# Baverne/VAE-CYCLEGAN-Implementation

Hardware: AMD Instinct MI355X
Metric: train images/sec (256x256 VAE-CycleGAN step) (higher is better)
Workload: dtype f32; 1 GPU; cyclevaegan unpaired, 3x256x256 synthetic summer<->winter, per-GPU batch 8, latent 64 (BASELINE.json configs[3]/[4]); per_gpu_batch=8, global_batch=8, image_size=256, latent_dim=64, parallelism=dp1, init=random (reference init statistics)

## Files before the change

vae-cyclegan-implementation_amd/csrc/conv_igemm.hip:

```cpp
#include "vcg_common.h"
#ifdef VCG_STAMP
#include <stdlib.h>
#endif

struct ConvP {
  const float* a;
  const float* b;
  const float* bias;
  float* out;
  int N, H, W, Cin, Cout, KH, KW, stride, pad, reflect, ups, act;
  int Hl, Wl, Ho, Wo, M, K;
  int cin4, cout4, cout_log;
  FastDiv fd_howo, fd_wo, fd_cin4, fd_cout4, fd_kw, fd_cin;
  int Hc, Wc, Mc, NB;
  FastDiv fd_hcwc, fd_wc;
  int ktiles_total, sk_len, sk_units, sk_ntn, sk_bm_shift, sk_bn_shift;
  int sk_ntr_pb;
  FastDiv fd_sklen;
  int ksplit, kt_per;
  float* slab;
  int adjoint;
  int src_pitch;
  uint32_t a_bytes, b_bytes;
  int dbl_mirror;
// ... 590 lines not shown
  f32x16 acc[MI][NI], tot[MI][NI];
#pragma unroll
  for (int i = 0; i < MI; ++i)
#pragma unroll
    for (int j = 0; j < NI; ++j)
#pragma unroll
      for (int e = 0; e < 16; ++e) acc[i][j][e] = tot[i][j][e] = 0.f;

  float4 va[AR], ve[AR], vb[BR];
  int nkt = (Kc + BK - 1) / BK;
  int kt0 = 0;
  if (p.ksplit > 1) {
    kt0 = kslice * p.kt_per;
    int kt1 = kt0 + p.kt_per;
    nkt = kt1 < nkt ? kt1 : nkt;
  }

  const __amdgpu_buffer_rsrc_t ra = make_srd(p.a, p.a_bytes), rb = make_srd(p.b, p.b_bytes);
  const int NONE = -(1 << 20);
  int eh[AR], ew[AR];
  bool edge[AR], any_edge = false;
#pragma unroll
  for (int r = 0; r < AR; ++r) {
    const int h = ph[r], w = pw[r];
    eh[r] = (h >= 1 && h <= p.pad) ? -h : (h >= p.Hl - 1 - p.pad && h <= p.Hl - 2) ? 2 * (p.Hl - 1) - h : NONE;
    ew[r] = (w >= 1 && w <= p.pad) ? -w : (w >= p.Wl - 1 - p.pad && w <= p.Wl - 2) ? 2 * (p.Wl - 1) - w : NONE;
    edge[r] = pv[r] && p.reflect && (eh[r] != NONE || ew[r] != NONE);
    any_edge = any_edge || edge[r];
    ve[r] = f4zero();
  }
  uint32_t rowoff[AR], xoff[AR][3], wbase[BR];
  int tap_cur = -1;

  auto load_tiles = [&](int kt) {
    const uint32_t g = (uint32_t)(kt * 8 + a_u);
    const bool kv = (int)(g * 4) < Kc;
    const uint32_t tapc = fd_div(g, p.fd_cout4);
    const int co = (int)(g - tapc * (uint32_t)p.cout4) * 4;
    if ((int)tapc != tap_cur) {
      tap_cur = (int)tapc;
      const int u = (int)tapc / nKW, v_ = (int)tapc % nKW;
      const int kh = kh0 + u * s, kw = kw0 + v_ * s;
      auto src = [&](int r, int qh, int qw) -> uint32_t {
        const int numh = qh - kh + p.pad, numw = qw - kw + p.pad;
        const int oh = numh >> sshift, ow = numw >> sshift;
        const bool ok = pv[r] && qh != NONE && qw != NONE && numh >= 0 && oh < p.Ho && numw >= 0 && ow < p.Wo;
        return ok ? (uint32_t)(((pnHo[r] + oh) * p.Wo + ow) * p.Cout) * 4u : VCG_OOB;
      };
#pragma unroll
      for (int r = 0; r < AR; ++r) {
        rowoff[r] = src(r, ph[r], pw[r]);
        if (any_edge) {
          xoff[r][0] = edge[r] ? src(r, eh[r], pw[r]) : VCG_OOB;
          xoff[r][1] = edge[r] ? src(r, ph[r], ew[r]) : VCG_OOB;
          xoff[r][2] = edge[r] ? src(r, eh[r], ew[r]) : VCG_OOB;
        }
      }
      const int tapfull = kh * p.KW + kw;
#pragma unroll
      for (int r = 0; r < BR; ++r) {
        const int J = n0 + a_row + 32 * r;
        wbase[r] = J < p.NB ? (uint32_t)((tapfull * p.NB + J) * p.Cout) * 4u : VCG_OOB;
      }
    }
    const uint32_t cb4 = (uint32_t)co * 4u;
#pragma unroll
    for (int r = 0; r < AR; ++r) va[r] = bload4(ra, (kv && rowoff[r] != VCG_OOB) ? rowoff[r] + cb4 : VCG_OOB);
    if (p.dbl_mirror) {
      const int u = tap_cur / nKW, v_ = tap_cur % nKW;
#pragma unroll
      for (int r = 0; r < AR; ++r)
        ve[r] = (pv[r] && kv) ? adjoint_extras(p, p.a, pnHo[r], ph[r], pw[r], kh0 + u * s, kw0 + v_ * s, co, sshift) : f4zero();
    } else if (any_edge) {
#pragma unroll
      for (int r = 0; r < AR; ++r) {
        float4 e = f4zero();
        if (edge[r] && kv) {
#pragma unroll
          for (int k = 0; k < 3; ++k)
            if (xoff[r][k] != VCG_OOB) f4add(e, bload4(ra, xoff[r][k] + cb4));
        }
        ve[r] = e;
      }
    }
#pragma unroll
    for (int r = 0; r < BR; ++r) vb[r] = bload4(rb, (kv && wbase[r] != VCG_OOB) ? wbase[r] + cb4 : VCG_OOB);
  };
  auto store_tiles = [&](int buf) {
#pragma unroll
    for (int r = 0; r < AR; ++r) {
      float* d = &As[buf][(a_row + 32 * r) * AS_STRIDE + a_u * 4];
      d[0] = va[r].x + ve[r].x; d[1] = va[r].y + ve[r].y; d[2] = va[r].z + ve[r].z; d[3] = va[r].w + ve[r].w;
    }
#pragma unroll
    for (int r = 0; r < BR; ++r) {
      float* d = &Bt[buf][(a_row + 32 * r) * AS_STRIDE + a_u * 4];
      d[0] = vb[r].x; d[1] = vb[r].y; d[2] = vb[r].z; d[3] = vb[r].w;
    }
  };

  if (kt0 < nkt) {
    load_tiles(kt0);
    store_tiles(0);
  }
  __syncthreads();
  VCG_STAMP_AT(1);
  for (int kt = kt0; kt < nkt; ++kt) {
    const int cur = (kt - kt0) & 1;
    const float* const Ac = As[cur];
    const float* const Bc = Bt[cur];
    if (kt + 1 < nkt) load_tiles(kt + 1);
    mma_ktile<MI, NI>(
        acc, [&](int kk, int i) { return Ac[(wm * (BM / WM) + i * 32 + l31) * AS_STRIDE + kk]; },
        [&](int kk, int j) { return Bc[(wn * (BN / WN) + j * 32 + l31) * AS_STRIDE + kk]; }, lh);
    if (((kt - kt0 + 1) & (FLUSH_TILES - 1)) == 0 && kt + 1 < nkt) flush_acc<MI, NI>(acc, tot);
    if (kt + 1 < nkt) store_tiles(cur ^ 1);
    __syncthreads();
  }
  VCG_STAMP_AT(2);
#pragma unroll
  for (int i = 0; i < MI; ++i)
#pragma unroll
    for (int j = 0; j < NI; ++j) acc[i][j] += tot[i][j];

  float* const dst = p.ksplit > 1 ? p.slab + (size_t)kslice * p.N * p.H * p.W * p.Cin : p.out;
#pragma unroll
  for (int j = 0; j < NI; ++j) {
    const int J = n0 + wn * (BN / WN) + j * 32 + l31;
    if (J >= p.NB) continue;
    int q = 0, c = J;
    if (p.ups == 2) { q = (int)fd_div((uint32_t)J, p.fd_cin); c = J - q * p.Cin; }
    const int qi = q >> 1, qj = q & 1;
#pragma unroll
    for (int i = 0; i < MI; ++i) {
#pragma unroll
      for (int e = 0; e < 16; ++e) {
        const int row = (e & 3) + 8 * (e >> 2) + 4 * lh;
        const uint32_t m = (uint32_t)(m0 + wm * (BM / WM) + i * 32 + row);
        if (m < (uint32_t)p.Mc) {
          uint32_t n = fd_div(m, p.fd_hcwc);
          uint32_t rem = m - n * (uint32_t)(p.Hc * p.Wc);
          uint32_t hq = fd_div(rem, p.fd_wc);
          uint32_t wq = rem - hq * (uint32_t)p.Wc;
          int h = (int)hq * s + ca, w = (int)wq * s + cb;
          size_t off = ((size_t)((int)n * p.H + h * p.ups + qi) * p.W + (w * p.ups + qj)) * p.Cin + c;
          dst[off] = acc[i][j][e];
        }
      }
    }
  }
  VCG_STAMP_AT(3);
}

template <int BN, int WN, bool BPL = (BN >= 64)>
__global__ __launch_bounds__(256, 2) void k_conv_dgrad_split(ConvP p) {
  VCG_STAMP_AT(0);
  constexpr int BM = 128, WM = 4 / WN;
  constexpr int MI = BM / (32 * WM), NI = BN / (32 * WN), AR = BM / 32, BR = BN / 32;
  __shared__ __attribute__((aligned(16))) unsigned char As[VCG_NP][BM * 64];
  __shared__ __attribute__((aligned(16))) unsigned char Bs[VCG_NP][BN * 64];
  const int tid = threadIdx.x, lane = tid & 63, wid = tid >> 6;
  const int wm = wid / WN, wn = wid % WN, l31 = lane & 31, lh = lane >> 5;
  const SplitScales sc = split_scales(p);
  const int m0 = blockIdx.x * BM, n0 = blockIdx.y * BN;
  const int a_row = tid >> 3, a_u = tid & 7;
  const int s = p.stride, sshift = s - 1;
  const int cls = (int)blockIdx.z % (s * s), kslice = (int)blockIdx.z / (s * s);
  const int ca = cls / s, cb = cls % s;
  const int kh0 = (ca + p.pad) % s, kw0 = (cb + p.pad) % s;
  const int nKH = (p.KH - kh0 + s - 1) / s, nKW = (p.KW - kw0 + s - 1) / s;
  const int Kc = nKH * nKW * p.Cout;

  int pnHo[AR], ph[AR], pw[AR];
  bool pv[AR];
#pragma unroll
  for (int r = 0; r < AR; ++r) {
    uint32_t m = (uint32_t)(m0 + a_row + 32 * r);
    pv[r] = m < (uint32_t)p.Mc;
    uint32_t n = fd_div(m, p.fd_hcwc);
    uint32_t rem = m - n * (uint32_t)(p.Hc * p.Wc);
    uint32_t hq = fd_div(rem, p.fd_wc);
    uint32_t wq = rem - hq * (uint32_t)p.Wc;
    pnHo[r] = (int)n * p.Ho;
    ph[r] = (int)hq * s + ca;
    pw[r] = (int)wq * s + cb;
  }

  f32x16 acc[MI][NI], lo[MI][NI];
#pragma unroll
  for (int i = 0; i < MI; ++i)
#pragma unroll
    for (int j = 0; j < NI; ++j)
#pragma unroll
      for (int e = 0; e < 16; ++e) acc[i][j][e] = lo[i][j][e] = 0.f;

  float4 va[AR], ve[AR], vb[BPL ? 1 : BR];
  constexpr int BP = BPL ? VCG_NP * BN / 64 : 1;
  const int b_q = tid & 3, b_r = tid >> 2;
  const int CB = p.Cout / 32;
  const uint32_t bsoff0 = (uint32_t)(b_r * 64 + ((b_q ^ ((b_r >> 2) & 3)) << 4));
  u32x4 vbp[BP];
  int nkt = (Kc + BK - 1) / BK;
  int kt0 = 0;
  if (p.ksplit > 1) {
    kt0 = kslice * p.kt_per;
    int kt1 = kt0 + p.kt_per;
    nkt = kt1 < nkt ? kt1 : nkt;
  }

  const __amdgpu_buffer_rsrc_t ra = make_srd(p.a, p.a_bytes), rb = make_srd(p.b, p.b_bytes);
  const int NONE = -(1 << 20);
  int eh[AR], ew[AR];
  bool edge[AR], any_edge = false;
#pragma unroll
  for (int r = 0; r < AR; ++r) {
    const int h = ph[r], w = pw[r];
    eh[r] = (h >= 1 && h <= p.pad) ? -h : (h >= p.Hl - 1 - p.pad && h <= p.Hl - 2) ? 2 * (p.Hl - 1) - h : NONE;
    ew[r] = (w >= 1 && w <= p.pad) ? -w : (w >= p.Wl - 1 - p.pad && w <= p.Wl - 2) ? 2 * (p.Wl - 1) - w : NONE;
    edge[r] = pv[r] && p.reflect && (eh[r] != NONE || ew[r] != NONE);
    any_edge = any_edge || edge[r];
    ve[r] = f4zero();
  }
  uint32_t rowoff[AR], xoff[AR][3], wbase[BR];
  int tap_cur = -1;

  auto load_tiles = [&](int kt) {
    const uint32_t g = (uint32_t)(kt * 8 + a_u);
    const bool kv = (int)(g * 4) < Kc;
    const uint32_t tapc = fd_div(g, p.fd_cout4);
    const int co = (int)(g - tapc * (uint32_t)p.cout4) * 4;
    if ((int)tapc != tap_cur) {
      tap_cur = (int)tapc;
      const int u = (int)tapc / nKW, v_ = (int)tapc % nKW;
      const int kh = kh0 + u * s, kw = kw0 + v_ * s;
      auto src = [&](int r, int qh, int qw) -> uint32_t {
        const int numh = qh - kh + p.pad, numw = qw - kw + p.pad;
        const int oh = numh >> sshift, ow = numw >> sshift;
        const bool ok = pv[r] && qh != NONE && qw != NONE && numh >= 0 && oh < p.Ho && numw >= 0 && ow < p.Wo;
        return ok ? (uint32_t)(((pnHo[r] + oh) * p.Wo + ow) * p.Cout) * 4u : VCG_OOB;
      };
#pragma unroll
      for (int r = 0; r < AR; ++r) {
        rowoff[r] = src(r, ph[r], pw[r]);
        if (any_edge) {
          xoff[r][0] = edge[r] ? src(r, eh[r], pw[r]) : VCG_OOB;
          xoff[r][1] = edge[r] ? src(r, ph[r], ew[r]) : VCG_OOB;
          xoff[r][2] = edge[r] ? src(r, eh[r], ew[r]) : VCG_OOB;
        }
      }
      const int tapfull = kh * p.KW + kw;
      if constexpr (!BPL) {
#pragma unroll
        for (int r = 0; r < BR; ++r) {
          const int J = n0 + a_row + 32 * r;
          wbase[r] = J < p.NB ? (uint32_t)((tapfull * p.NB + J) * p.Cout) * 4u : VCG_OOB;
        }
      }
    }
    const uint32_t cb4 = (uint32_t)co * 4u;
#pragma unroll
    for (int r = 0; r < AR; ++r) va[r] = bload4(ra, (kv && rowoff[r] != VCG_OOB) ? rowoff[r] + cb4 : VCG_OOB);
    if (p.dbl_mirror) {
      const int u = tap_cur / nKW, v_ = tap_cur % nKW;
#pragma unroll
      for (int r = 0; r < AR; ++r)
        ve[r] = (pv[r] && kv) ? adjoint_extras(p, p.a, pnHo[r], ph[r], pw[r], kh0 + u * s, kw0 + v_ * s, co, sshift) : f4zero();
    } else if (any_edge) {
#pragma unroll
      for (int r = 0; r < AR; ++r) {
        float4 e = f4zero();
        if (edge[r] && kv) {
#pragma unroll
          for (int k = 0; k < 3; ++k)
            if (xoff[r][k] != VCG_OOB) f4add(e, bload4(ra, xoff[r][k] + cb4));
        }
        ve[r] = e;
      }
    }
    if constexpr (BPL) {
      const int tk = (kt * 32) / p.Cout, cob = (kt * 32 - tk * p.Cout) >> 5;
      const int tf = (kh0 + (tk / nKW) * s) * p.KW + (kw0 + (tk % nKW) * s);
      const bool kvt = kt * 32 < Kc;
#pragma unroll
      for (int j = 0; j < BP; ++j) {
        const int J = n0 + b_r + 64 * (j / VCG_NP);
        const uint32_t off = (kvt && J < p.NB) ? (uint32_t)((((size_t)tf * p.NB + J) * CB + cob) * VCG_PBYTES + (j % VCG_NP) * 64 + b_q * 16) : VCG_OOB;
        vbp[j] = __builtin_amdgcn_raw_buffer_load_b128(rb, (int)off, 0, 0);
      }
    } else {
#pragma unroll
      for (int r = 0; r < BR; ++r) vb[r] = bload4(rb, (kv && wbase[r] != VCG_OOB) ? wbase[r] + cb4 : VCG_OOB);
    }
  };
  uint32_t soff[AR > BR ? AR : BR];
#pragma unroll
  for (int i = 0; i < (AR > BR ? AR : BR); ++i) {
    const int r = a_row + 32 * i;
    soff[i] = (uint32_t)(r * 64 + (((a_u >> 1) ^ ((r >> 2) & 3)) << 4) + ((a_u & 1) << 3));
  }
  auto store_tiles = [&]() {
#pragma unroll
    for (int r = 0; r < AR; ++r) {
      const float4 v = make_float4(va[r].x + ve[r].x, va[r].y + ve[r].y, va[r].z + ve[r].z, va[r].w + ve[r].w);
      uint2 h, l;
      split4h(v, sc.inv_a, h, l);
      *reinterpret_cast<uint2*>(&As[0][soff[r]]) = h;
      *reinterpret_cast<uint2*>(&As[1][soff[r]]) = l;
    }
    if constexpr (BPL) {
#pragma unroll
      for (int j = 0; j < BP; ++j) *reinterpret_cast<u32x4*>(&Bs[j % VCG_NP][bsoff0 + 4096 * (j / VCG_NP)]) = vbp[j];
    } else {
#pragma unroll
      for (int r = 0; r < BR; ++r) {
        uint2 h, l;
        split4h(vb[r], sc.inv_b, h, l);
        *reinterpret_cast<uint2*>(&Bs[0][soff[r]]) = h;
        *reinterpret_cast<uint2*>(&Bs[1][soff[r]]) = l;
      }
    }
  };
  uint32_t fa[MI], fb[NI];
  int sa[MI], sb[NI];
#pragma unroll
  for (int i = 0; i < MI; ++i) { const int r = wm * (BM / WM) + i * 32 + l31; fa[i] = (uint32_t)(r * 64); sa[i] = (r >> 2) & 3; }
#pragma unroll
  for (int j = 0; j < NI; ++j) { const int r = wn * (BN / WN) + j * 32 + l31; fb[j] = (uint32_t)(r * 64); sb[j] = (r >> 2) & 3; }

  if (kt0 < nkt) {
    load_tiles(kt0);
    store_tiles();
  }
  __syncthreads();
  VCG_STAMP_AT(1);
  for (int kt = kt0; kt < nkt; ++kt) {
    if (kt + 1 < nkt) load_tiles(kt + 1);
    split_mma_ktile<MI, NI>(acc, lo, As, Bs, fa, fb, sa, sb, lh);
    __syncthreads();
    if (kt + 1 < nkt) {
      store_tiles();
      __syncthreads();
    }
  }
  VCG_STAMP_AT(2);
#pragma unroll
  for (int i = 0; i < MI; ++i)
#pragma unroll
    for (int j = 0; j < NI; ++j) acc[i][j] += lo[i][j];

  float* const dst = p.ksplit > 1 ? p.slab + (size_t)kslice * p.N * p.H * p.W * p.Cin : p.out;
#pragma unroll
  for (int j = 0; j < NI; ++j) {
    const int J = n0 + wn * (BN / WN) + j * 32 + l31;
    if (J >= p.NB) continue;
    int q = 0, c = J;
    if (p.ups == 2) { q = (int)fd_div((uint32_t)J, p.fd_cin); c = J - q * p.Cin; }
    const int qi = q >> 1, qj = q & 1;
#pragma unroll
    for (int i = 0; i < MI; ++i) {
#pragma unroll
      for (int e = 0; e < 16; ++e) {
        const int row = (e & 3) + 8 * (e >> 2) + 4 * lh;
        const uint32_t m = (uint32_t)(m0 + wm * (BM / WM) + i * 32 + row);
        if (m < (uint32_t)p.Mc) {
          uint32_t n = fd_div(m, p.fd_hcwc);
          uint32_t rem = m - n * (uint32_t)(p.Hc * p.Wc);
          uint32_t hq = fd_div(rem, p.fd_wc);
          uint32_t wq = rem - hq * (uint32_t)p.Wc;
          int h = (int)hq * s + ca, w = (int)wq * s + cb;
          size_t off = ((size_t)((int)n * p.H + h * p.ups + qi) * p.W + (w * p.ups + qj)) * p.Cin + c;
          dst[off] = acc[i][j][e] * sc.out;
        }
      }
    }
  }
  VCG_STAMP_AT(3);
}

__device__ __forceinline__ int sk_logical_wg() {
  const uint32_t nwg = gridDim.x, gid = blockIdx.x;
  const uint32_t q = nwg >> 3, r = nwg & 7, xcd = gid & 7;
  return (int)((xcd < r ? xcd * (q + 1) : r * (q + 1) + (xcd - r) * q) + (gid >> 3));
}

template <int BM, int BN, int NT = 256>
__global__ __launch_bounds__(NT) void k_conv_wgrad(ConvP p) {
  VCG_STAMP_AT(0);
  constexpr int WR = NT / 128;
  constexpr int MI = BM / (32 * WR), NI = BN / 64;
  constexpr int RQ = BM / 4, PS = NT / RQ, AP = BK / PS, BE = (BK * BN / 4) / NT;
  __shared__ __attribute__((aligned(16))) float Xs[2][BK * BM];
  __shared__ __attribute__((aligned(16))) float Ds[2][BK * BN];
  const int tid = threadIdx.x, lane = tid & 63, wid = tid >> 6;
  const int wm = wid >> 1, wn = wid & 1, l31 = lane & 31, lh = lane >> 5;
  const int rq = tid % RQ, ps = tid / RQ;
  const uint32_t bstep = (uint32_t)(BK * p.Cout * 4);
  const bool row_aligned = !p.adjoint && (p.Wo % BK) == 0;

  const int wg = sk_logical_wg();
  int unit = wg * p.sk_len;
  int unit_end = unit + p.sk_len;
  if (unit_end > p.sk_units) unit_end = p.sk_units;
  while (unit < unit_end) {
  const int tile = unit / p.ktiles_total;
  const int kt_begin = unit - tile * p.ktiles_total;
  int kt_end = kt_begin + (unit_end - unit);
  if (kt_end > p.ktiles_total) kt_end = p.ktiles_total;
  const int tr = tile / p.sk_ntn;
  const int zb = tr / p.sk_ntr_pb;
  const int r0 = (tr - zb * p.sk_ntr_pb) * BM, n0 = (tile - tr * p.sk_ntn) * BN;
  const __amdgpu_buffer_rsrc_t ra = make_srd(p.a + (size_t)zb * p.a_bstride, p.a_bytes),
                               rb = make_srd(p.b + (size_t)zb * p.b_bstride, p.b_bytes);

  const int R = r0 + rq * 4;
  const bool rv = R < p.K;
  int kh, kw, ii, jj, c;
  decode_tap(p, (uint32_t)(R >> 2), kh, kw, ii, jj, c);

  f32x16 acc[MI][NI];
#pragma unroll
  for (int i = 0; i < MI; ++i)
#pragma unroll
    for (int j = 0; j < NI; ++j)
#pragma unroll
      for (int e = 0; e < 16; ++e) acc[i][j][e] = 0.f;

  float4 va[AP], vb[BE];

  uint32_t sm[AP];
  int sn[AP], soh[AP], sow[AP];
#pragma unroll
  for (int a = 0; a < AP; ++a) {
    uint32_t m = (uint32_t)(kt_begin * BK + ps + PS * a);
    uint32_t n = fd_div(m, p.fd_howo);
    uint32_t rem = m - n * (uint32_t)(p.Ho * p.Wo);
    uint32_t oh = fd_div(rem, p.fd_wo);
    sm[a] = m; sn[a] = (int)n; soh[a] = (int)oh; sow[a] = (int)(rem - oh * (uint32_t)p.Wo);
  }
  uint32_t boff[BE];
#pragma unroll
  for (int e = 0; e < BE; ++e) {
    int idx = tid + NT * e;
    int pp = idx / (BN / 4), j4 = idx % (BN / 4);
    const int co = n0 + j4 * 4;
    boff[e] = co < p.Cout ? (uint32_t)(((kt_begin * BK + pp) * p.Cout + co) * 4) : VCG_OOB;
  }

  auto load_tiles = [&](int ) {
    if (row_aligned) {
      const int n = sn[0], oh = soh[0];
      int ih = oh * p.stride - p.pad + kh;
      bool okr = rv && sm[0] < (uint32_t)p.M;
      if (p.reflect) ih = reflect_idx(ih, p.Hl);
      else okr = okr && ih >= 0 && ih < p.Hl;
      const uint32_t rowbase = (uint32_t)(((n * p.H + ih * p.ups + ii) * p.W + jj) * p.Cin + c) * 4u;
      const uint32_t colstep = (uint32_t)(p.ups * p.Cin) * 4u;
#pragma unroll
      for (int a = 0; a < AP; ++a) {
        int iw = sow[a] * p.stride - p.pad + kw;
        bool ok = okr;
        if (p.reflect) iw = reflect_idx(iw, p.Wl);
        else ok = ok && iw >= 0 && iw < p.Wl;
        va[a] = bload4(ra, ok ? rowbase + (uint32_t)iw * colstep : VCG_OOB);
        sm[a] += BK;
        sow[a] += BK;
        if (sow[a] >= p.Wo) { sow[a] -= p.Wo; ++soh[a]; if (soh[a] >= p.Ho) { soh[a] = 0; ++sn[a]; } }
      }
    } else {
#pragma unroll
      for (int a = 0; a < AP; ++a) {
        const int n = sn[a], oh = soh[a], ow = sow[a];
        if (p.adjoint) {
          float4 v = f4zero();
          if (rv && sm[a] < (uint32_t)p.M) {
            float4 ex;
            adjoint_gather(p, p.a, n * p.Ho, oh, ow, kh, kw, 0, 0, v, ex);
            f4add(v, ex);
          }
          va[a] = v;
        } else {
          int ih = oh * p.stride - p.pad + kh, iw = ow * p.stride - p.pad + kw;
          bool ok = rv && sm[a] < (uint32_t)p.M;
          if (p.reflect) {
            ih = reflect_idx(ih, p.Hl);
            iw = reflect_idx(iw, p.Wl);
          } else {
            ok = ok && (ih >= 0) && (ih < p.Hl) && (iw >= 0) && (iw < p.Wl);
          }
          const uint32_t off = ok ? (uint32_t)(((n * p.H + ih * p.ups + ii) * p.W + (iw * p.ups + jj)) * p.Cin + c) * 4u : VCG_OOB;
          va[a] = bload4(ra, off);
        }
        sm[a] += BK;
        sow[a] += BK;
        while (sow[a] >= p.Wo) { sow[a] -= p.Wo; ++soh[a]; }
        while (soh[a] >= p.Ho) { soh[a] -= p.Ho; ++sn[a]; }
      }
    }
#pragma unroll
    for (int e = 0; e < BE; ++e) {
      vb[e] = bload4(rb, boff[e]);
      if (boff[e] != VCG_OOB) boff[e] += bstep;
    }
  };
  auto store_tiles = [&](int buf) {
#pragma unroll
    for (int a = 0; a < AP; ++a)
      *reinterpret_cast<float4*>(&Xs[buf][(ps + PS * a) * BM + rq * 4]) = va[a];
#pragma unroll
    for (int e = 0; e < BE; ++e) {
      int idx = tid + NT * e;
      int pp = idx / (BN / 4), j4 = idx % (BN / 4);
      *reinterpret_cast<float4*>(&Ds[buf][pp * BN + j4 * 4]) = vb[e];
    }
  };

  if (kt_begin < kt_end) {
    load_tiles(kt_begin);
    store_tiles(0);
  }
  __syncthreads();
  VCG_STAMP_AT(1);
  for (int kt = kt_begin; kt < kt_end; ++kt) {
    const int cur = (kt - kt_begin) & 1;
    const float* const Xc = Xs[cur];
    const float* const Dc = Ds[cur];
    if (kt + 1 < kt_end) load_tiles(kt + 1);
    mma_ktile<MI, NI>(
        acc, [&](int kk, int i) { return Xc[kk * BM + wm * (BM / WR) + i * 32 + l31]; },
        [&](int kk, int j) { return Dc[kk * BN + wn * (BN / 2) + j * 32 + l31]; }, lh);
// ... 847 lines not shown
  int bm, bn, nsplit, kt_per;
  fwd_plan(g, bm, bn, nsplit, kt_per);
  return bm == 128 && bn >= 64 && nsplit == 1 && wft_wanted(g) && (g.Ho * g.Wo) % 128 == 0;
}

static int conv_fwd_impl(const float* x, const float* wf, const float* bias, float* y, const int32_t* cd, void* ws,
                         size_t ws_bytes, void* stream, double* in_part, const VcgInStatsOut* stats, float* saved = nullptr,
                         const VcgPre* pre = nullptr) {
  const uint64_t x_handle = vcg_take_hint_x();
  (void)vcg_take_hint_dy();
  ConvGeom g;
  if (vcg_conv_geom(cd, &g, "vcg_conv_fwd")) return -1;
  VCG_CHECK_ARG(x && wf && y, "vcg_conv_fwd: null pointer");
  if (pre && pre->mean)
    VCG_CHECK_ARG(!vcg_thin_fold_ok(g) && !vcg_thin_fwd_ok(g) && vcg_wino_fwd_ok(g),
                  "vcg_conv_fwd_in_pre: this geometry has no normalising gather (ask vcg_conv_pre_ok first)");
  if (vcg_thin_fold_ok(g)) return vcg_thin_fold_fwd(g, x, wf + wf_floats(g), vcg_pack_amax(g, wf), bias, y, ws, ws_bytes, (hipStream_t)stream, x_handle);
  if (vcg_thin_fwd_ok(g)) return vcg_thin_fwd(g, x, wf, bias, y, (hipStream_t)stream);
  if (vcg_thinin_fwd_ok(g)) {
    if (vcg_thinin_fwd(g, x, wf, vcg_pack_amax(g, wf), bias, y, in_part, (hipStream_t)stream, x_handle)) return -2;
    if (in_part)
      return vcg_in_finalize(in_part, stats->mean, stats->rstd, g.N, stats->HW, g.Cout, vcg_thinin_nchunk(g), stats->eps, (hipStream_t)stream);
    return 0;
  }
  if (vcg_wino_fwd_ok(g))
    return vcg_wino_fwd(g, x, wf + wf_floats(g), vcg_pack_amax(g, wf), bias, y, ws, ws_bytes, (hipStream_t)stream, in_part, stats, saved, x_handle,
                        pre);
  if (fwd_slab_ok(g))
    return vcg_slab_fwd(g, x, wf + wft_offset(g), wft_floats(g) * 4, vcg_pack_amax(g, wf), bias, y, in_part, stats, (hipStream_t)stream, x_handle);
  ConvP p; fill_params(g, p);
  if (in_part) {
    p.in_part = in_part;
    p.in_nchunk = g.Ho * g.Wo / 128;
  }
  p.a = x; p.b = wf; p.bias = bias; p.out = y;
  {
    const unsigned long long ab = (unsigned long long)g.N * g.H * g.W * g.Cin * 4, bb = (unsigned long long)g.K * g.Cout * 4;
    VCG_CHECK_ARG(ab < (1ull << 31) && bb < (1ull << 31), "vcg_conv_fwd: tensor extents must stay below 2 GiB");
    p.a_bytes = (uint32_t)ab; p.b_bytes = (uint32_t)bb;
  }
  int bm, bn, nsplit, kt_per;
  fwd_plan(g, bm, bn, nsplit, kt_per);
  if (nsplit > 1) {
    VCG_CHECK_ARG(ws && ws_bytes >= vcg_conv_fwd_workspace(cd), "vcg_conv_fwd: workspace too small (%zu)", ws_bytes);
    p.ksplit = nsplit; p.kt_per = kt_per; p.slab = (float*)ws;
  }
  dim3 grid((g.M + bm - 1) / bm, (g.Cout + bn - 1) / bn, nsplit);
  hipStream_t st = (hipStream_t)stream;
  const double gemm_flops = 2.0 * g.M * (double)g.K * g.Cout;
  if (bm == 128 && bn >= 64 && wft_wanted(g)) {
    p.b = wf + wft_offset(g);
    p.b_bytes = (uint32_t)(wft_floats(g) * 4);
    if (vcg_operand_amax(x, (size_t)g.N * g.H * g.W * g.Cin, x_handle, 0, st, &p.amax_a)) return -2;
    p.amax_b = vcg_amax_stored(vcg_pack_amax(g, wf));
    VcgProfScope prof(bn == 128 ? "k_conv_fwd_split<128>" : "k_conv_fwd_split<64>", gemm_flops, st);
    if (bn == 128) hipLaunchKernelGGL((k_conv_fwd_split<128>), grid, dim3(256), 0, st, p);
    else hipLaunchKernelGGL((k_conv_fwd_split<64>), grid, dim3(256), 0, st, p);
  } else {
    VcgProfScope prof("k_conv_fwd<fp32 MFMA>", gemm_flops, st);
    if (bm == 128 && bn == 128 && g.K <= 2048) hipLaunchKernelGGL((k_conv_fwd<128, 128, 2, false>), grid, dim3(256), 0, st, p);
    else DISPATCH_FWD(bm, bn, grid, st, p);
  }
  if (nsplit > 1)
    hipLaunchKernelGGL(k_splitk_finish, dim3(ew_grid((size_t)g.M * g.Cout / 4)), dim3(256), 0, st, (const float*)ws, bias,
                       y, (size_t)g.M, g.Cout, nsplit, g.cout_log, g.act);
  VCG_LAUNCH_CHECK("vcg_conv_fwd");
  if (in_part) return vcg_in_finalize(in_part, stats->mean, stats->rstd, g.N, stats->HW, g.Cout, p.in_nchunk, stats->eps, st);
  return 0;
}

extern "C" int vcg_conv_fwd(const float* x, const float* wf, const float* bias, float* y,
                            const int32_t* cd, void* ws, size_t ws_bytes, void* stream) {
  return conv_fwd_impl(x, wf, bias, y, cd, ws, ws_bytes, stream, nullptr, nullptr);
}

static size_t fwd_in_conv_ws(const int32_t* cd) { return (vcg_conv_fwd_workspace(cd) + 255) / 256 * 256; }

extern "C" size_t vcg_conv_fwd_in_workspace(const int32_t* cd) {
  ConvGeom g;
  if (vcg_conv_geom(cd, &g, "vcg_conv_fwd_in_workspace")) return 0;
  size_t part;
  const bool thinin = !vcg_thin_fold_ok(g) && !vcg_thin_fwd_ok(g) && vcg_thinin_fwd_ok(g);
  if (thinin) part = (size_t)g.N * vcg_thinin_nchunk(g) * g.Cout * 2 * sizeof(double);
  else if (vcg_wino_fwd_ok(g)) part = vcg_wino_fwd_stats_doubles(g) * sizeof(double);
  else if (fwd_slab_ok(g) && vcg_slab_fwd_stats_ok(g)) part = (size_t)g.N * vcg_slab_fwd_nchunk(g) * g.Cout * 2 * sizeof(double);
  else if (fwd_tile_stats_ok(g)) part = (size_t)g.N * (g.Ho * g.Wo / 128) * g.Cout * 2 * sizeof(double);
  else part = vcg_in_workspace(g.N, g.Ho * g.Wo, g.Cout);
  return fwd_in_conv_ws(cd) + part;
}

extern "C" size_t vcg_conv_saved_floats(const int32_t* cd) {
  ConvGeom g;
  if (vcg_conv_geom(cd, &g, "vcg_conv_saved_floats")) return 0;
  return vcg_wino_fwd_ok(g) ? vcg_wino_saved_floats(g) : 0;
}

static int conv_fwd_in_impl(const float* x, const float* wf, const float* bias, float* y, float* mean, float* rstd,
                            float eps, float* saved, const int32_t* cd, void* ws, size_t ws_bytes, void* stream, const VcgPre* pre);
extern "C" int vcg_conv_fwd_in(const float* x, const float* wf, const float* bias, float* y, float* mean, float* rstd,
                               float eps, float* saved, const int32_t* cd, void* ws, size_t ws_bytes, void* stream) {
  return conv_fwd_in_impl(x, wf, bias, y, mean, rstd, eps, saved, cd, ws, ws_bytes, stream, nullptr);
}
extern "C" int vcg_conv_pre_ok(const int32_t* cd) {
  ConvGeom g;
  if (vcg_conv_geom(cd, &g, "vcg_conv_pre_ok")) return 0;
  return (!vcg_thin_fold_ok(g) && !vcg_thin_fwd_ok(g) && vcg_wino_fwd_ok(g)) ? 1 : 0;
}
extern "C" int vcg_conv_fwd_in_pre(const float* t_prev, const float* pre_mean, const float* pre_rstd, int pre_act, const float* wf,
                                   const float* bias, float* y, float* mean, float* rstd, float eps, float* saved, const int32_t* cd,
                                   void* ws, size_t ws_bytes, void* stream) {
  VCG_CHECK_ARG(pre_mean && pre_rstd, "vcg_conv_fwd_in_pre: null statistics");
  VCG_CHECK_ARG(pre_act >= VCG_ACT_NONE && pre_act <= VCG_ACT_SIGMOID, "vcg_conv_fwd_in_pre: bad activation %d", pre_act);
  const VcgPre pre = {pre_mean, pre_rstd, pre_act};
  (void)vcg_take_hint_x();
  return conv_fwd_in_impl(t_prev, wf, bias, y, mean, rstd, eps, saved, cd, ws, ws_bytes, stream, &pre);
}
static int conv_fwd_in_impl(const float* x, const float* wf, const float* bias, float* y, float* mean, float* rstd,
                            float eps, float* saved, const int32_t* cd, void* ws, size_t ws_bytes, void* stream, const VcgPre* pre) {
  ConvGeom g;
  if (vcg_conv_geom(cd, &g, "vcg_conv_fwd_in")) return -1;
  VCG_CHECK_ARG((mean == nullptr) == (rstd == nullptr), "vcg_conv_fwd_in: mean and rstd go together");
  if (saved && !vcg_conv_saved_floats(cd)) saved = nullptr;
  if (!mean) {
    VCG_CHECK_ARG(ws_bytes >= vcg_conv_fwd_workspace(cd), "vcg_conv_fwd_in: workspace too small (%zu)", ws_bytes);
    return conv_fwd_impl(x, wf, bias, y, cd, ws, ws_bytes, stream, nullptr, nullptr, saved, pre);
  }
  VCG_CHECK_ARG(ws, "vcg_conv_fwd_in: null pointer");
  VCG_CHECK_ARG(ws_bytes >= vcg_conv_fwd_in_workspace(cd), "vcg_conv_fwd_in: workspace too small (%zu)", ws_bytes);
  const size_t cws = fwd_in_conv_ws(cd);
  double* part = reinterpret_cast<double*>(static_cast<char*>(ws) + cws);
  const bool thinin = !vcg_thin_fold_ok(g) && !vcg_thin_fwd_ok(g) && vcg_thinin_fwd_ok(g);
  const bool fused = thinin || vcg_wino_fwd_ok(g) || (fwd_slab_ok(g) && vcg_slab_fwd_stats_ok(g)) || fwd_tile_stats_ok(g);
  const VcgInStatsOut stats = {mean, rstd, g.Ho * g.Wo, eps};
  if (conv_fwd_impl(x, wf, bias, y, cd, ws, cws, stream, fused ? part : nullptr, &stats, saved, pre)) return -1;
  if (fused) return 0;
  return vcg_in_stats_pass(y, mean, rstd, g.N, g.Ho * g.Wo, g.Cout, eps, part, ws_bytes - cws, (hipStream_t)stream);
}

static int dgrad_setup(const ConvGeom& g, ConvP& p, int& bm, int& bn, int& nsplit, int& kt_per) {
  p.Hc = g.Hl / g.stride; p.Wc = g.Wl / g.stride; p.Mc = g.N * p.Hc * p.Wc;
  p.NB = g.ups * g.ups * g.Cin;
  p.fd_hcwc = make_fastdiv((uint32_t)(p.Hc * p.Wc));
  p.fd_wc = make_fastdiv((uint32_t)p.Wc);
  const int s = g.stride;
  gemm_plan(p.Mc, p.NB, (g.KH * g.KW * g.Cout + BK - 1) / BK, s == 1, bm, bn, nsplit, kt_per, 1, true);
  if (s > 1 && g.KH % s == 0 && g.KW % s == 0) {
    const long long wgs = ((p.Mc + bm - 1) / bm) * ((p.NB + bn - 1) / bn) * s * s;
    if (wgs < 384)
      gemm_plan(p.Mc, p.NB, ((g.KH / s) * (g.KW / s) * g.Cout + BK - 1) / BK, true, bm, bn, nsplit, kt_per, s * s, true);
  }
  return 0;
}

static bool fwd_reads_wf(const ConvGeom& g) {
  if (vcg_thin_fold_ok(g)) return false;
  if (vcg_thin_fwd_ok(g) || vcg_thinin_fwd_ok(g)) return true;
  if (vcg_wino_fwd_ok(g) || fwd_slab_ok(g)) return false;
  int bm, bn, nsplit, kt_per;
  fwd_plan(g, bm, bn, nsplit, kt_per);
  return !(bm == 128 && bn >= 64 && wft_wanted(g));
}
static bool dgrad_reads_wf(const ConvGeom& g) {
  if (g.Hl % g.stride || g.Wl % g.stride) return true;
  if (vcg_thin_fold_dgrad_ok(g)) return false;
  if (vcg_thin_dgrad_ok(g)) return true;
  if (vcg_wino_dgrad_ok(g) || dgrad_slab_ok(g)) return false;
  ConvP p; fill_params(g, p);
  int bm, bn, nsplit, kt_per;
  dgrad_setup(g, p, bm, bn, nsplit, kt_per);
  return !(bm == 128 && bn >= 64 && wfd_wanted(g));
}
extern "C" int vcg_conv_reads_wf(const int32_t* cd) {
  ConvGeom g;
  if (vcg_conv_geom(cd, &g, "vcg_conv_reads_wf")) return 1;
  return (fwd_reads_wf(g) || dgrad_reads_wf(g)) ? 1 : 0;
}

extern "C" size_t vcg_conv_dgrad_workspace(const int32_t* cd) {
  ConvGeom g;
  if (vcg_conv_geom(cd, &g, "vcg_conv_dgrad_workspace")) return 0;
  if (g.Hl % g.stride || g.Wl % g.stride) return 0;
  if (vcg_thin_fold_dgrad_ok(g)) return vcg_thin_fold_dgrad_workspace(g);
  if (vcg_thin_dgrad_ok(g)) return vcg_thin_dgrad_workspace(g);
  if (vcg_wino_dgrad_ok(g)) return vcg_wino_dgrad_workspace(g);
  if (dgrad_slab_ok(g)) return vcg_slab_dgrad_workspace(g);
  ConvP p; fill_params(g, p);
  int bm, bn, nsplit, kt_per;
  dgrad_setup(g, p, bm, bn, nsplit, kt_per);
  return nsplit > 1 ? (size_t)nsplit * g.N * g.H * g.W * g.Cin * sizeof(float) + 256 : 0;
}

extern "C" int vcg_conv_dgrad(const float* dy, const float* wf, float* dx, const int32_t* cd, void* ws,
                              size_t ws_bytes, void* stream) {
  (void)vcg_take_hint_x();
  const uint64_t dy_handle = vcg_take_hint_dy();
  ConvGeom g;
  if (vcg_conv_geom(cd, &g, "vcg_conv_dgrad")) return -1;
  VCG_CHECK_ARG(dy && wf && dx, "vcg_conv_dgrad: null pointer");
  VCG_CHECK_ARG(g.Hl % g.stride == 0 && g.Wl % g.stride == 0, "vcg_conv_dgrad: input %dx%d not divisible by stride", g.Hl, g.Wl);
  VCG_CHECK_ARG(g.stride == 1 || g.ups == 1, "vcg_conv_dgrad: stride 2 with ups 2 unsupported");
  if (vcg_thin_fold_dgrad_ok(g)) return vcg_thin_fold_dgrad(g, dy, wf + wkd_offset(g), vcg_pack_amax(g, wf), dx, ws, ws_bytes, (hipStream_t)stream, dy_handle);
  if (vcg_thin_dgrad_ok(g)) return vcg_thin_dgrad(g, dy, wf, dx, ws, ws_bytes, (hipStream_t)stream);
  if (vcg_wino_dgrad_ok(g))
    return vcg_wino_dgrad(g, dy, wf + wf_floats(g) + wino_u_floats(g), vcg_pack_amax(g, wf), dx, ws, ws_bytes, (hipStream_t)stream, dy_handle);
  if (dgrad_slab_ok(g))
    return vcg_slab_dgrad(g, dy, wf + wfd_offset(g), wfd_floats(g) * 4, vcg_pack_amax(g, wf), dx, ws, ws_bytes, (hipStream_t)stream, dy_handle);
  ConvP p; fill_params(g, p);
  p.a = dy; p.b = wf; p.out = dx;
  {
    const unsigned long long ab = (unsigned long long)g.M * g.Cout * 4, bb = (unsigned long long)g.K * g.Cout * 4;
    VCG_CHECK_ARG(ab < (1ull << 31) && bb < (1ull << 31), "vcg_conv_dgrad: tensor extents must stay below 2 GiB");
    p.a_bytes = (uint32_t)ab; p.b_bytes = (uint32_t)bb;
  }
  {
    auto dbl = [&](int L) { int lo = 1 > L - 1 - g.pad ? 1 : L - 1 - g.pad, hi = g.pad < L - 2 ? g.pad : L - 2; return lo <= hi; };
    p.dbl_mirror = g.reflect && (dbl(g.Hl) || dbl(g.Wl));
  }
  int bm, bn, nsplit, kt_per;
  dgrad_setup(g, p, bm, bn, nsplit, kt_per);
  if (nsplit > 1) {
    VCG_CHECK_ARG(ws && ws_bytes >= vcg_conv_dgrad_workspace(cd), "vcg_conv_dgrad: workspace too small (%zu)", ws_bytes);
    p.ksplit = nsplit; p.kt_per = kt_per; p.slab = (float*)ws;
  }
  dim3 grid((p.Mc + bm - 1) / bm, (p.NB + bn - 1) / bn, nsplit * g.stride * g.stride);
  hipStream_t st = (hipStream_t)stream;
  {
    const double gemm_flops = 2.0 * g.M * (double)g.K * g.Cout;
    const bool planes = bm == 128 && bn >= 64 && wfd_wanted(g);
    if (planes) { p.b = wf + wfd_offset(g); p.b_bytes = (uint32_t)(wfd_floats(g) * 4); }
    const bool nopl64 = !planes && bm == 128 && bn == 64 && g.Cout % 4 == 0;
    const bool split = planes || bn == 32 || nopl64;
    if (split) {
      if (vcg_operand_amax(dy, (size_t)g.M * g.Cout, dy_handle, g.reflect ? 4 : 0, st, &p.amax_a)) return -2;
      p.amax_b = vcg_amax_stored(vcg_pack_amax(g, wf));
    }
    VcgProfScope prof(!split ? "k_conv_dgrad<fp32 MFMA>" : bn == 128 ? "k_conv_dgrad_split<128, 2>" : bn == 64 ? "k_conv_dgrad_split<64, 2>"
                                                                                                             : "k_conv_dgrad_split<32, 1>",
                      gemm_flops, st);
    if (planes) {
      if (bn == 128) hipLaunchKernelGGL((k_conv_dgrad_split<128, 2>), grid, dim3(256), 0, st, p);
      else hipLaunchKernelGGL((k_conv_dgrad_split<64, 2>), grid, dim3(256), 0, st, p);
    } else if (bn == 32) hipLaunchKernelGGL((k_conv_dgrad_split<32, 1>), grid, dim3(256), 0, st, p);
    else if (nopl64) hipLaunchKernelGGL((k_conv_dgrad_split<64, 2, false>), grid, dim3(256), 0, st, p);
    else DISPATCH_DGRAD(bm, bn, grid, st, p);
  }
  if (nsplit > 1)
    hipLaunchKernelGGL(k_splitk_finish, dim3(ew_grid((size_t)g.N * g.H * g.W * g.Cin / 4)), dim3(256), 0, st,
                       (const float*)ws, (const float*)nullptr, dx, (size_t)g.N * g.H * g.W, g.Cin, nsplit, g.Cin,
                       (int)VCG_ACT_NONE);
  VCG_LAUNCH_CHECK("vcg_conv_dgrad");
  return 0;
}

struct WgradPlan { int bm, bn, grid, len, parts, total, ntr, ntn; };
static WgradPlan wgrad_plan(const ConvGeom& g, int batches = 1) {
  WgradPlan best_p = {};
  const int total = (g.M + BK - 1) / BK;
  struct Cand { int bm, bn, resident; double t_step; };
  const Cand cands[4] = {{256, 128, 1, 4.3}, {128, 128, 2, 5.1}, {128, 64, 3, 4.7}, {64, 64, 5, 4.8}};
  double best = 1e30;
  int force = 0;
#ifdef VCG_STAMP
  { const char* e = getenv("VCG_WGRAD_BM"); force = e ? atoi(e) : 0; }
#endif
  for (int ci = 0; ci < 4; ++ci) {
    const Cand& c = cands[ci];
    if (force ? c.bm != force : c.bm == 256) continue;
    if (c.bn == 128 && g.Cout <= 64) continue;
    if (c.bm >= 128 && g.K <= 64) continue;
    if (c.bm == 256 && g.K < 512) continue;
    if (batches > 1 && g.K % c.bm) continue;
    const int ntr = ((g.K + c.bm - 1) / c.bm) * batches, ntn = (g.Cout + c.bn - 1) / c.bn;
    const long long tiles = (long long)ntr * ntn, units = tiles * total;
    if (units >= (1LL << 30)) continue;
    const long long slots = 256LL * c.resident;
    long long len = (units + slots - 1) / slots;
    if (len < 8) len = units < 8 ? units : 8;
    const long long grid = (units + len - 1) / len;
    const int parts = (int)((total + len - 1) / len) + 1;
    double t = (double)len * c.t_step + (double)(grid + tiles) * c.bm * c.bn * 8.0 / 3.0e6;
    if (t < best * 0.97) {
      best = t;
      best_p = {c.bm, c.bn, (int)grid, (int)len, parts, total, ntr, ntn};
    }
  }
  return best_p;
}

static const int kMaxDirectSlabs = 24;

static void colsum_plan(const ConvGeom& g, int& tc, int& cgroups, int& rows, int& nchunk) {
  int c4 = g.Cout / 4;
  tc = 1;
  while (tc * 2 <= c4 && tc * 2 <= 256) tc *= 2;
  cgroups = (c4 + tc - 1) / tc;
  int tp = 256 / tc;
  long long want = 512 / cgroups;
  if (want < 1) want = 1;
  long long r = (g.M + want - 1) / want;
  if (r < 4LL * tp) r = 4LL * tp;
  rows = (int)r;
  nchunk = (g.M + rows - 1) / rows;
}

static bool wgrad_swapped_ok(const ConvGeom& g);
static ConvGeom swapped_geom(const ConvGeom& g);

static ConvGeom wino_gemm_geom(const ConvGeom& g, int T) {
  ConvGeom q = {};
  q.N = 1; q.H = 1; q.W = T; q.Cin = g.ups * g.ups * g.Cin; q.Cout = g.Cout; q.KH = q.KW = 1; q.stride = 1; q.pad = 0;
  q.reflect = 0; q.ups = 1; q.act = VCG_ACT_NONE; q.cin_log = q.Cin; q.cout_log = g.Cout;
  q.Hl = 1; q.Wl = T; q.Ho = 1; q.Wo = T; q.M = T; q.K = q.Cin; q.taps = 1;
  return q;
}
size_t vcg_wino_wgrad_core_workspace(const ConvGeom& g, int T) {
  const ConvGeom q = wino_gemm_geom(g, T);
  const WgradPlan wp = wgrad_plan(q, 16);
  return (size_t)wp.parts * 16 * q.K * q.Cout * sizeof(float) + 256;
}
int vcg_wino_wgrad_core(const ConvGeom& g, const float* V, const float* dM, int T, float* gw_oihw, void* ws, size_t ws_bytes,
                        hipStream_t st, const VcgAmax& amax_v, const VcgAmax& amax_dm) {
  const ConvGeom q = wino_gemm_geom(g, T);
  const WgradPlan wp = wgrad_plan(q, 16);
  VCG_CHECK_ARG(wp.grid > 0, "vcg_conv_wgrad: no launch plan for the Winograd path");
  VCG_CHECK_ARG(ws_bytes >= vcg_wino_wgrad_core_workspace(g, T), "vcg_conv_wgrad: Winograd slab workspace too small");
  ConvP p; fill_params(q, p);
  p.a = V; p.b = dM; p.out = (float*)ws;
  p.amax_a = amax_v; p.amax_b = amax_dm;
  p.a_planes = 1;
  VCG_CHECK_ARG(wp.bm == 128 && q.K % 32 == 0, "vcg_conv_wgrad: pre-split V needs the split-operand tile");
  p.a_bytes = (uint32_t)((size_t)T * q.K * 4); p.b_bytes = (uint32_t)((size_t)T * q.Cout * 4);
  p.nbatch = 16; p.a_bstride = (uint32_t)((size_t)T * q.K); p.b_bstride = (uint32_t)((size_t)T * q.Cout);
  p.ktiles_total = wp.total; p.sk_len = wp.len; p.sk_units = wp.ntr * wp.ntn * wp.total; p.sk_ntn = wp.ntn;
  p.sk_bm_shift = wp.bm == 256 ? 8 : wp.bm == 128 ? 7 : 6; p.sk_bn_shift = wp.bn == 128 ? 7 : 6;
  p.sk_ntr_pb = wp.ntr / 16;
  p.fd_sklen = make_fastdiv((uint32_t)wp.len);
  dim3 grid(wp.grid);
  {
    VcgProfScope prof(wp.bm == 128 ? (wp.bn == 128 ? "k_conv_wgrad_split<128>" : "k_conv_wgrad_split<64>") : "k_conv_wgrad<fp32 MFMA>",
                      2.0 * 16 * (double)T * q.K * q.Cout, st);
    if (wp.bm == 128 && wp.bn == 128) hipLaunchKernelGGL(k_conv_wgrad_split<128>, grid, dim3(256), 0, st, p);
    else if (wp.bm == 128 && wp.bn == 64) hipLaunchKernelGGL(k_conv_wgrad_split<64>, grid, dim3(256), 0, st, p);
    else if (wp.bm == 64 && wp.bn == 128) hipLaunchKernelGGL((k_conv_wgrad<64, 128>), grid, dim3(256), 0, st, p);
    else hipLaunchKernelGGL((k_conv_wgrad<64, 64>), grid, dim3(256), 0, st, p);
  }
  VCG_LAUNCH_CHECK("vcg_conv_wgrad(winograd gemm)");
  hipLaunchKernelGGL(k_wino_wgrad_reduce, dim3(g.Cout / 64, (g.Cin + 7) / 8, g.ups * g.ups), dim3(256), 0, st,
                     (const float*)ws, gw_oihw, p, g.Cin, g.ups, g.cin_log, g.cout_log);
  VCG_LAUNCH_CHECK("vcg_conv_wgrad(winograd reduce)");
  return 0;
}

int vcg_wino_wgrad_reduce_one(const ConvGeom& g, const float* dU, float* gw_oihw, hipStream_t st) {
  const ConvGeom q = wino_gemm_geom(g, 32);
  ConvP p; fill_params(q, p);
  p.nbatch = 16;
  p.ktiles_total = 1; p.sk_len = 1; p.sk_ntn = 1; p.sk_bm_shift = 30; p.sk_bn_shift = 30;
  p.fd_sklen = make_fastdiv(1u);
  hipLaunchKernelGGL(k_wino_wgrad_reduce, dim3(g.Cout / 64, (g.Cin + 7) / 8, g.ups * g.ups), dim3(256), 0, st, dU, gw_oihw, p, g.Cin,
                     g.ups, g.cin_log, g.cout_log);
  VCG_LAUNCH_CHECK("vcg_conv_wgrad(winograd reduce)");
  return 0;
}

extern "C" size_t vcg_conv_wgrad_workspace(const int32_t* cd) {
  ConvGeom g;
  if (vcg_conv_geom(cd, &g, "vcg_conv_wgrad_workspace")) return 0;
  const ConvGeom gorig = g;
  int tc, cgroups, rows, nchunk;
  colsum_plan(gorig, tc, cgroups, rows, nchunk);
  size_t cols = (size_t)nchunk * gorig.Cout * sizeof(float);
  if (vcg_wino_wgrad_ok(g)) return ((vcg_wino_wgrad_workspace(g) + 255) / 256) * 256 + cols + 1024;
  if (wgrad_ring_ok(g)) return ((vcg_ring_wgrad_workspace(g) + 255) / 256) * 256 + cols + 1024;
  if (wgrad_swapped_ok(g)) g = swapped_geom(g);
  const WgradPlan wp = wgrad_plan(g);
  const int nsplit = wp.parts;
  size_t slabs = (size_t)nsplit * g.K * g.Cout * sizeof(float);
  size_t groups = (size_t)16 * g.K * g.Cout * sizeof(float);
  return slabs + groups + cols + 1024;
}

static bool wgrad_swapped_ok(const ConvGeom& g) {
  return g.Cout == 4 && g.stride == 1 && g.ups == 1 && g.Ho == g.H && g.Wo == g.W && g.Cin >= 32;
}
static ConvGeom swapped_geom(const ConvGeom& g) {
  ConvGeom s = g;
  s.Cin = 4; s.Cout = g.Cin; s.cin_log = g.cout_log; s.cout_log = g.cin_log;
  s.taps = g.KH * g.KW; s.K = s.taps * 4; s.M = g.N * g.H * g.W; s.act = 0;
  return s;
}

static int launch_colsum(const ConvGeom& gorig, const float* dy, float* gbias, float* part, hipStream_t st) {
  int tc, cgroups, rows, nchunk;
  colsum_plan(gorig, tc, cgroups, rows, nchunk);
  hipLaunchKernelGGL(k_colsum_partial, dim3(cgroups, nchunk), dim3(256), 0, st, dy, part, gorig.M, gorig.Cout, rows, tc);
// ... 101 lines not shown
```

Baseline: 247.0 images/s.

## Add stride-2 4x4 dgrad kernel that reuses a shared dy window across taps

Adds a specialised split-precision dgrad kernel for stride-2, 4x4, pad-1 convolutions. Each output-channel chunk of dy is loaded once into a padded shared-memory window of up to 288 rows. The four kernel taps of each parity class then read that window at shifted row offsets, instead of re-gathering dy with im2col for every tap. B tiles are double-buffered. This cuts global loads and address math for the A operand, at the cost of a larger LDS footprint and possible occupancy pressure. A host check limits it to geometries where the window fits.

Result: slower. 243.3 images/s (-1.5%).

```diff
diff --git a/vae-cyclegan-implementation_amd/csrc/conv_igemm.hip b/vae-cyclegan-implementation_amd/csrc/conv_igemm.hip
--- a/vae-cyclegan-implementation_amd/csrc/conv_igemm.hip
+++ b/vae-cyclegan-implementation_amd/csrc/conv_igemm.hip
@@ -766,8 +766,8 @@
   VCG_STAMP_AT(3);
 }
 
-template <int BN, int WN, bool BPL = (BN >= 64)>
-__global__ __launch_bounds__(256, 2) void k_conv_dgrad_split(ConvP p) {
+template <int BN, int WN, bool BPL>
+__device__ __forceinline__ void dgrad_split_body(const ConvP& p) {
   VCG_STAMP_AT(0);
   constexpr int BM = 128, WM = 4 / WN;
   constexpr int MI = BM / (32 * WM), NI = BN / (32 * WN), AR = BM / 32, BR = BN / 32;
@@ -989,6 +989,198 @@
     }
   }
   VCG_STAMP_AT(3);
+}
+
+constexpr int S2_ROWS = 288;
+template <int BN, int WN, bool BPL>
+__device__ __forceinline__ void dgrad_split_s2_body(const ConvP& p) {
+  VCG_STAMP_AT(0);
+  constexpr int BM = 128, WM = 4 / WN;
+  constexpr int MI = BM / (32 * WM), NI = BN / (32 * WN), BR = BN / 32;
+  constexpr int AQ = S2_ROWS / 32;
+  __shared__ __attribute__((aligned(16))) unsigned char As[VCG_NP][S2_ROWS * 64];
+  __shared__ __attribute__((aligned(16))) unsigned char Bs[2][VCG_NP][BN * 64];
+  const int tid = threadIdx.x, lane = tid & 63, wid = tid >> 6;
+  const int wm = wid / WN, wn = wid % WN, l31 = lane & 31, lh = lane >> 5;
+  const SplitScales sc = split_scales(p);
+  const int m0 = blockIdx.x * BM, n0 = blockIdx.y * BN;
+  const int a_row = tid >> 3, a_u = tid & 7;
+  const int cls = (int)blockIdx.z & 3, kslice = (int)blockIdx.z >> 2;
+  const int ca = cls >> 1, cb = cls & 1;
+  const int Wp = p.Wc + 1, Hp = p.Hc + 1;
+  auto padded = [&](int mm) -> int {
+    const uint32_t m = (uint32_t)mm;
+    const uint32_t n = fd_div(m, p.fd_hcwc);
+    const uint32_t rem = m - n * (uint32_t)(p.Hc * p.Wc);
+    const uint32_t hq = fd_div(rem, p.fd_wc);
+    return ((int)n * Hp + (int)hq) * Wp + (int)(rem - hq * (uint32_t)p.Wc);
+  };
+  const int mlast = (m0 + BM < p.Mc ? m0 + BM : p.Mc) - 1;
+  const int P0 = padded(m0);
+  const int wrows = padded(mlast) - P0 + Wp + 2;
+  const int q0 = P0 + (ca - 1) * Wp + (cb - 1);
+
+  const __amdgpu_buffer_rsrc_t ra = make_srd(p.a, p.a_bytes), rb = make_srd(p.b, p.b_bytes);
+  uint32_t goff[AQ], soff[AQ];
+#pragma unroll
+  for (int a = 0; a < AQ; ++a) {
+    const int lrow = a_row + 32 * a, q = q0 + lrow;
+    const uint32_t qq = q > 0 ? (uint32_t)q : 0u;
+    const uint32_t R = qq / (uint32_t)Wp, ow = qq - R * (uint32_t)Wp;
+    const uint32_t n = R / (uint32_t)Hp, oh = R - n * (uint32_t)Hp;
+    const bool ok = lrow < wrows && q >= 0 && (int)ow < p.Wc && (int)oh < p.Hc && (int)n < p.N;
+    goff[a] = ok ? (uint32_t)((((int)n * p.Ho + (int)oh) * p.Wo + (int)ow) * p.Cout + a_u * 4) * 4u : VCG_OOB;
+    soff[a] = lrow < wrows ? (uint32_t)(lrow * 64 + (((a_u >> 1) ^ ((lrow >> 2) & 3)) << 4) + ((a_u & 1) << 3)) : VCG_OOB;
+  }
+  int prow[MI];
+#pragma unroll
+  for (int i = 0; i < MI; ++i) {
+    const int m = m0 + wm * (BM / WM) + i * 32 + l31;
+    prow[i] = padded(m < mlast ? m : mlast) - P0;
+  }
+  uint32_t fb[NI];
+  int sb[NI];
+#pragma unroll
+  for (int j = 0; j < NI; ++j) { const int r = wn * (BN / WN) + j * 32 + l31; fb[j] = (uint32_t)(r * 64); sb[j] = (r >> 2) & 3; }
+
+  constexpr int BP = BPL ? VCG_NP * BN / 64 : 1;
+  constexpr int NBO = BPL ? BN / 64 : BR;
+  const int b_q = tid & 3, b_r = tid >> 2;
+  const int CB = p.Cout / 32;
+  const uint32_t bsoff0 = (uint32_t)(b_r * 64 + ((b_q ^ ((b_r >> 2) & 3)) << 4));
+  uint32_t boff[NBO], bsoff[BR];
+#pragma unroll
+  for (int h = 0; h < NBO; ++h) {
+    const int J = BPL ? n0 + b_r + 64 * h : n0 + a_row + 32 * h;
+    boff[h] = J >= p.NB ? VCG_OOB : BPL ? (uint32_t)J * (uint32_t)(CB * VCG_PBYTES) + (uint32_t)(b_q * 16)
+                                        : (uint32_t)J * (uint32_t)(p.Cout * 4) + (uint32_t)(a_u * 16);
+  }
+#pragma unroll
+  for (int r = 0; r < BR; ++r) {
+    const int row = a_row + 32 * r;
+    bsoff[r] = (uint32_t)(row * 64 + (((a_u >> 1) ^ ((row >> 2) & 3)) << 4) + ((a_u & 1) << 3));
+  }
+  const uint32_t tap_bytes = (uint32_t)p.NB * (uint32_t)p.Cout * 4u;
+
+  f32x16 acc[MI][NI], lo[MI][NI];
+#pragma unroll
+  for (int i = 0; i < MI; ++i)
+#pragma unroll
+    for (int j = 0; j < NI; ++j)
+#pragma unroll
+      for (int e = 0; e < 16; ++e) acc[i][j][e] = lo[i][j][e] = 0.f;
+
+  int nkt = 4 * CB, kt0 = 0;
+  if (p.ksplit > 1) {
+    kt0 = kslice * p.kt_per;
+    const int kt1 = kt0 + p.kt_per;
+    nkt = kt1 < nkt ? kt1 : nkt;
+  }
+  float4 va[AQ], vb[BPL ? 1 : BR];
+  u32x4 vbp[BP];
+  auto load_a = [&](int chunk) {
+#pragma unroll
+    for (int a = 0; a < AQ; ++a)
+      if (a * 32 < wrows) va[a] = bload4(ra, goff[a] != VCG_OOB ? goff[a] + (uint32_t)chunk * 128u : VCG_OOB);
+  };
+  auto store_a = [&]() {
+#pragma unroll
+    for (int a = 0; a < AQ; ++a)
+      if (a * 32 < wrows && soff[a] != VCG_OOB) {
+        uint2 h, l;
+        split4h(va[a], sc.inv_a, h, l);
+        *reinterpret_cast<uint2*>(&As[0][soff[a]]) = h;
+        *reinterpret_cast<uint2*>(&As[1][soff[a]]) = l;
+      }
+  };
+  auto load_b = [&](int s) {
+    const int chunk = s >> 2, u = (s >> 1) & 1, v = s & 1;
+    const uint32_t o = (uint32_t)((1 - ca + 2 * u) * p.KW + (1 - cb + 2 * v)) * tap_bytes + (uint32_t)chunk * (uint32_t)VCG_PBYTES;
+    if constexpr (BPL) {
+#pragma unroll
+      for (int j = 0; j < BP; ++j)
+        vbp[j] = __builtin_amdgcn_raw_buffer_load_b128(rb, (int)(boff[j / VCG_NP] != VCG_OOB ? boff[j / VCG_NP] + o + (uint32_t)(j % VCG_NP) * 64u : VCG_OOB), 0, 0);
+    } else {
+#pragma unroll
+      for (int r = 0; r < BR; ++r) vb[r] = bload4(rb, boff[r] != VCG_OOB ? boff[r] + o : VCG_OOB);
+    }
+  };
+  auto store_b = [&](int buf) {
+    if constexpr (BPL) {
+#pragma unroll
+      for (int j = 0; j < BP; ++j) *reinterpret_cast<u32x4*>(&Bs[buf][j % VCG_NP][bsoff0 + 4096 * (j / VCG_NP)]) = vbp[j];
+    } else {
+#pragma unroll
+      for (int r = 0; r < BR; ++r) {
+        uint2 h, l;
+        split4h(vb[r], sc.inv_b, h, l);
+        *reinterpret_cast<uint2*>(&Bs[buf][0][bsoff[r]]) = h;
+        *reinterpret_cast<uint2*>(&Bs[buf][1][bsoff[r]]) = l;
+      }
+    }
+  };
+
+  if (kt0 < nkt) {
+    load_a(kt0 >> 2);
+    load_b(kt0);
+    store_a();
+    store_b(0);
+  }
+  __syncthreads();
+  VCG_STAMP_AT(1);
+  for (int s = kt0; s < nkt; ++s) {
+    const int buf = (s - kt0) & 1;
+    const bool more = s + 1 < nkt;
+    if (more) load_b(s + 1);
+    if (((s & 3) == 0 || s == kt0) && (s | 3) + 1 < nkt) load_a((s >> 2) + 1);
+    const int toff = (1 - ((s >> 1) & 1)) * Wp + (1 - (s & 1));
+    uint32_t fa[MI];
+    int sa[MI];
+#pragma unroll
+    for (int i = 0; i < MI; ++i) { const int r = prow[i] + toff; fa[i] = (uint32_t)(r * 64); sa[i] = (r >> 2) & 3; }
+    split_mma_ktile<MI, NI>(acc, lo, As, Bs[buf], fa, fb, sa, sb, lh);
+    if (more) store_b(buf ^ 1);
+    if (more && ((s + 1) & 3) == 0) {
+      __syncthreads();
+      store_a();
+    }
+    __syncthreads();
+  }
+  VCG_STAMP_AT(2);
+#pragma unroll
+  for (int i = 0; i < MI; ++i)
+#pragma unroll
+    for (int j = 0; j < NI; ++j) acc[i][j] += lo[i][j];
+
+  float* const dst = p.ksplit > 1 ? p.slab + (size_t)kslice * p.N * p.H * p.W * p.Cin : p.out;
+#pragma unroll
+  for (int j = 0; j < NI; ++j) {
+    const int J = n0 + wn * (BN / WN) + j * 32 + l31;
+    if (J >= p.NB) continue;
+#pragma unroll
+    for (int i = 0; i < MI; ++i) {
+#pragma unroll
+      for (int e = 0; e < 16; ++e) {
+        const int row = (e & 3) + 8 * (e >> 2) + 4 * lh;
+        const uint32_t m = (uint32_t)(m0 + wm * (BM / WM) + i * 32 + row);
+        if (m < (uint32_t)p.Mc) {
+          const uint32_t n = fd_div(m, p.fd_hcwc);
+          const uint32_t rem = m - n * (uint32_t)(p.Hc * p.Wc);
+          const uint32_t hq = fd_div(rem, p.fd_wc);
+          const uint32_t wq = rem - hq * (uint32_t)p.Wc;
+          const int h = (int)hq * 2 + ca, w = (int)wq * 2 + cb;
+          dst[((size_t)((int)n * p.H + h) * p.W + w) * p.Cin + J] = acc[i][j][e] * sc.out;
+        }
+      }
+    }
+  }
+  VCG_STAMP_AT(3);
+}
+
+template <int BN, int WN, bool BPL = (BN >= 64), bool S2 = false>
+__global__ __launch_bounds__(256, 2) void k_conv_dgrad_split(ConvP p) {
+  if constexpr (S2) dgrad_split_s2_body<BN, WN, BPL>(p);
+  else dgrad_split_body<BN, WN, BPL>(p);
 }
 
 __device__ __forceinline__ int sk_logical_wg() {
@@ -2142,6 +2334,14 @@
   return 0;
 }
 
+static bool dgrad_s2_window_ok(const ConvGeom& g, const ConvP& p) {
+  if (!(g.stride == 2 && g.KH == 4 && g.KW == 4 && g.pad == 1 && !g.reflect && g.ups == 1 && g.Cout % 32 == 0)) return false;
+  if (p.Hc != g.Ho || p.Wc != g.Wo) return false;
+  const long long rows = (p.Mc < 128 ? p.Mc : 128) - 1, hw = (long long)p.Hc * p.Wc;
+  const long long span = rows + (rows + p.Wc - 1) / p.Wc + ((rows + hw - 1) / hw) * (p.Wc + 1);
+  return span + p.Wc + 3 <= S2_ROWS;
+}
+
 static bool fwd_reads_wf(const ConvGeom& g) {
   if (vcg_thin_fold_ok(g)) return false;
   if (vcg_thin_fwd_ok(g) || vcg_thinin_fwd_ok(g)) return true;
@@ -2227,10 +2427,14 @@
     VcgProfScope prof(!split ? "k_conv_dgrad<fp32 MFMA>" : bn == 128 ? "k_conv_dgrad_split<128, 2>" : bn == 64 ? "k_conv_dgrad_split<64, 2>"
                                                                                                              : "k_conv_dgrad_split<32, 1>",
                       gemm_flops, st);
+    const bool s2 = dgrad_s2_window_ok(g, p);
     if (planes) {
-      if (bn == 128) hipLaunchKernelGGL((k_conv_dgrad_split<128, 2>), grid, dim3(256), 0, st, p);
+      if (bn == 128 && s2) hipLaunchKernelGGL((k_conv_dgrad_split<128, 2, true, true>), grid, dim3(256), 0, st, p);
+      else if (bn == 128) hipLaunchKernelGGL((k_conv_dgrad_split<128, 2>), grid, dim3(256), 0, st, p);
+      else if (s2) hipLaunchKernelGGL((k_conv_dgrad_split<64, 2, true, true>), grid, dim3(256), 0, st, p);
       else hipLaunchKernelGGL((k_conv_dgrad_split<64, 2>), grid, dim3(256), 0, st, p);
     } else if (bn == 32) hipLaunchKernelGGL((k_conv_dgrad_split<32, 1>), grid, dim3(256), 0, st, p);
+    else if (nopl64 && s2) hipLaunchKernelGGL((k_conv_dgrad_split<64, 2, false, true>), grid, dim3(256), 0, st, p);
     else if (nopl64) hipLaunchKernelGGL((k_conv_dgrad_split<64, 2, false>), grid, dim3(256), 0, st, p);
     else DISPATCH_DGRAD(bm, bn, grid, st, p);
   }
```
